# WU-CVGL/VicaSplat

Hardware: AMD Instinct MI355X
Metric: scenes/sec (8-view 256x256) encode+rasterize (higher is better)
Workload: dtype f32 (f32 activations; products as 3 x f16 MFMA on hi+lo operand pairs, f32 accumulate); 1 GPU; re10k_8view full pipeline fwd: ViT-L encoder+decoder+DPT heads -> 524288 Gaussians/scene, 12 target views/scene rasterized at 256x256; scenes_per_gpu=24, context_views=8, target_views=12, parallelism=scene-sharded x1 (no collective)

## Files before the change

### include/vicasplat_hip.h

```cpp
#ifndef VICASPLAT_HIP_H
#define VICASPLAT_HIP_H

#include <stddef.h>
#include <stdint.h>

#ifdef __cplusplus
extern "C" {
#endif

typedef void *vs_stream_t;

const char *vs_last_error(void);
int vs_abi_version(void);

typedef struct VsRasterIn {
    int32_t num_cameras;
    int32_t num_scenes;
    int32_t P;
    int32_t sh_degree;
    int32_t sh_coeffs;
    int32_t width, height;
    int32_t flags;
    const float *means3D;
    const float *cov3D;
// ... 63 lines not shown

int vs_rope2d(void *tokens, const int64_t *pos, int32_t B, int32_t N, int32_t H, int32_t D, int64_t sB, int64_t sN,
              float base, float fwd, int32_t dtype, vs_stream_t stream);


int vs_split_pack_weight(const float *w, int64_t ldw, void *out, int64_t ldo, int32_t N, int32_t K, int32_t scale_exp, vs_stream_t stream);

int vs_gemm_split(const float *A, const void *Wp, float acc_scale, const float *bias, float *out, const float *gate, const float *resid,
                  int32_t M, int32_t N, int32_t K, int32_t lda, int32_t ldw, int32_t ldo, int32_t epilogue, int32_t grp_in, int32_t grp_out,
                  int32_t grp_off, int32_t gate_rows, int32_t gate_ld, int32_t a_grp_in, int32_t a_grp_out, int32_t a_grp_off,
                  const int32_t *pos, const uint8_t *kind, int32_t C, float base2d, float theta1d, vs_stream_t stream);

int vs_conv3x3_split_res2_nhwc(const float *in, const void *wp, float acc_scale, const float *bias, const float *residual, const float *residual2,
                               float *out, int32_t Nimg, int32_t Hin, int32_t Win, int32_t Cin, int32_t Cout, int32_t stride, int32_t relu_in,
                               int32_t relu_out, vs_stream_t stream);
int vs_gemm_split_packed(const void *Ap, const void *Wp, float acc_scale, const float *bias, float *out, const float *gate, const float *resid,
                         int32_t M, int32_t N, int32_t K, int32_t lda, int32_t ldw, int32_t ldo, int32_t epilogue, int32_t grp_in, int32_t grp_out,
                         int32_t grp_off, int32_t gate_rows, int32_t gate_ld, int32_t a_grp_in, int32_t a_grp_out, int32_t a_grp_off,
                         const int32_t *pos, const uint8_t *kind, int32_t C, float base2d, float theta1d, vs_stream_t stream);
int vs_conv7x7_rgb_split_nhwc(const float *in_padded, const void *wp, float acc_scale, const float *bias, float *out, int32_t Nimg, int32_t H,
                              int32_t W, int32_t Hp, int32_t Wp, int32_t Cout, vs_stream_t stream);
int vs_conv7x7_rgb_split_up_nhwc(const float *in_padded, const void *wp, float acc_scale, const float *bias, const float *up_src, void *out_packed,
                                 int32_t Nimg, int32_t H, int32_t W, int32_t Hp, int32_t Wp, int32_t Cout, vs_stream_t stream);

int vs_conv3x3_head_dot_split_nhwc(const float *in, const void *wp, float acc_scale, const float *bias, const float *w2, const float *bias2,
                                   float *out2, int32_t Nimg, int32_t H, int32_t W, int32_t Cin, int32_t C2, int32_t ld2, int32_t relu_in,
                                   int32_t relu_out, vs_stream_t stream);

int vs_conv3x3_head1x1_split_nhwc(const float *in, const void *wp, float acc_scale, const float *bias, const void *w2p, float acc_scale2,
                                  const float *bias2, float *out2, int32_t Nimg, int32_t H, int32_t W, int32_t Cin, int32_t C2, int32_t C2pad,
// ... 155 lines not shown
```

### vicasplat_amd/_lib.py

```python
from __future__ import annotations

import ctypes as C
import os
import subprocess
import threading

import torch

_HERE = os.path.dirname(os.path.abspath(__file__))
_SO = os.environ.get("VICASPLAT_HIP_LIB") or os.path.join(_HERE, "libvicasplat_hip.so")
_lock = threading.Lock()
ABI_VERSION = 8
_lib = None

VS_BUF_GEOM, VS_BUF_RECT, VS_BUF_CLAMPED, VS_BUF_TILE_RANGES, VS_BUF_TILE_CURSOR, VS_BUF_KEYS, VS_BUF_POINT_LIST, \
    VS_BUF_SORT_SCRATCH, VS_BUF_FINAL_T, VS_BUF_N_CONTRIB, VS_BUF_MISC, VS_BUF_DEPTH, VS_BUF_CHECKPOINT, VS_BUF_COUNT = range(14)
VS_RASTER_COUNT_TOUCHED = 1
VS_RASTER_SAVE_FOR_BACKWARD = 2
VS_RASTER_SH_RGB_MAJOR = 4
VS_RASTER_COV_3X3 = 8

AllocFn = C.CFUNCTYPE(C.c_void_p, C.c_void_p, C.c_int32, C.c_size_t)


class VsRasterIn(C.Structure):
    _fields_ = [
        ("num_cameras", C.c_int32), ("num_scenes", C.c_int32), ("P", C.c_int32), ("sh_degree", C.c_int32),
# ... 121 lines not shown
            L.vs_linear_f32.argtypes = [vp, i64, vp, i64, vp, vp, i64, i32, i32, i32, i32, vp]
            L.vs_silu_cast.restype = C.c_int
            L.vs_silu_cast.argtypes = [vp, vp, i64, i32, vp]
            L.vs_conv3x3_head1x1_nhwc.restype = C.c_int
            L.vs_conv3x3_head1x1_nhwc.argtypes = [vp, vp, vp, vp, vp, vp] + [i32] * 11 + [vp]
            L.vs_split_pack_weight.restype = C.c_int
            L.vs_split_pack_weight.argtypes = [vp, i64, vp, i64, i32, i32, i32, vp]
            L.vs_gemm_split.restype = C.c_int
            L.vs_gemm_split.argtypes = [vp, vp, f32, vp, vp, vp, vp] + [i32] * 15 + [vp, vp, i32, f32, f32, vp]
            L.vs_gemm_split_packed.restype = C.c_int
            L.vs_gemm_split_packed.argtypes = [vp, vp, f32, vp, vp, vp, vp] + [i32] * 15 + [vp, vp, i32, f32, f32, vp]
            L.vs_conv3x3_split_nhwc.restype = C.c_int
            L.vs_conv3x3_split_nhwc.argtypes = [vp, vp, f32, vp, vp, vp] + [i32] * 8 + [vp]
            L.vs_conv3x3_split_res2_nhwc.restype = C.c_int
            L.vs_conv3x3_split_res2_nhwc.argtypes = [vp, vp, f32, vp, vp, vp, vp] + [i32] * 8 + [vp]
            L.vs_conv3x3_head1x1_split_nhwc.restype = C.c_int
            L.vs_conv3x3_head1x1_split_nhwc.argtypes = [vp, vp, f32, vp, vp, f32, vp, vp] + [i32] * 8 + [vp]
            L.vs_conv3x3_head_dot_split_nhwc.restype = C.c_int
            L.vs_conv3x3_head_dot_split_nhwc.argtypes = [vp, vp, f32, vp, vp, vp, vp] + [i32] * 8 + [vp]
            L.vs_conv7x7_rgb_split_nhwc.restype = C.c_int
            L.vs_conv7x7_rgb_split_nhwc.argtypes = [vp, vp, f32, vp, vp, i32, i32, i32, i32, i32, i32, vp]
            L.vs_conv7x7_rgb_split_up_nhwc.restype = C.c_int
            L.vs_conv7x7_rgb_split_up_nhwc.argtypes = [vp, vp, f32, vp, vp, vp, i32, i32, i32, i32, i32, i32, vp]
            L.vs_upsample2x_nhwc.restype = C.c_int
            L.vs_upsample2x_nhwc.argtypes = [vp, vp, vp, i32, i32, i32, i32, i32, i32, vp]
            L.vs_probe_mfma_rate.restype = C.c_int
            L.vs_probe_mfma_rate.argtypes = [vp, vp, i32, C.POINTER(C.c_double), vp]
            L.vs_transpose_f32.restype = C.c_int
            L.vs_transpose_f32.argtypes = [vp, i64, vp, i64, i32, i32, i32, i32, i32, i32, i32, i32, vp, vp]
            L.vs_gemm_wgrad_split_atn.restype = C.c_int
# ... 67 lines not shown
```

### vicasplat_amd/csrc/api.hip

```cpp
#include "common.h"

namespace vs {
static thread_local char g_err[512] = "";
void set_error(const char *fmt, ...) {
    va_list ap;
    va_start(ap, fmt);
    vsnprintf(g_err, sizeof(g_err), fmt, ap);
    va_end(ap);
}
}

extern "C" const char *vs_last_error(void) { return vs::g_err; }
extern "C" int vs_abi_version(void) { return 8; }

namespace {
typedef _Float16 half8p __attribute__((ext_vector_type(8)));
typedef float f4p __attribute__((ext_vector_type(4)));
__global__ void __launch_bounds__(256) mfma_rate_kernel(const half8p *__restrict__ in, float *__restrict__ out, int iters) {
    const int t = blockIdx.x * 256 + threadIdx.x;
    half8p a[4], b[4];
#pragma unroll
    for (int i = 0; i < 4; ++i) { a[i] = in[(t * 8 + i) & 65535]; b[i] = in[(t * 8 + 4 + i) & 65535]; }
    f4p c[16];
#pragma unroll
    for (int i = 0; i < 16; ++i) c[i] = f4p{0.f, 0.f, 0.f, 0.f};
    for (int it = 0; it < iters; ++it) {
#pragma unroll
        for (int i = 0; i < 4; ++i)
// ... 19 lines not shown
```

### vicasplat_amd/csrc/conv.hip

```cpp
#include "gemm256.h"

#include <cstdlib>

__device__ __attribute__((aligned(128))) unsigned short vs_zero_page[64] = {0};

namespace {

struct ConvArgs {
    const unsigned short *in;
    const unsigned short *w;
    const float *bias;
    const unsigned short *res;
    unsigned short *out;
    int Nimg, H, W, Cin, Cout;
    int relu_in, relu_out;
    int Hin, Win, stride;
    const unsigned short *w2;
    const float *bias2;
    unsigned short *out2;
    int C2, C2pad, ld2;
    float acc_scale;
    float acc_scale2;
    int a_packed;
    const float *res2;
    int korder;
};

static int conv_korder() {
    static const int v = [] { const char *e = getenv("VS_CONV_KORDER"); return e ? atoi(e) : 1; }();
    return v;
}

template <int BF16, int MI>
__device__ __forceinline__ void conv_epilogue(const ConvArgs &g, f4 (&acc)[MI][4], int mw0, int nbase, int M, void *, int, int lane) {
    const int mrow = lane & 15, c4 = (lane >> 4) * 4;
    if constexpr (BF16 == kDtSplit) {
#pragma unroll
        for (int i = 0; i < MI; ++i)
#pragma unroll
            for (int j = 0; j < 4; ++j) acc[i][j] *= g.acc_scale;
// ... 46 lines not shown
                } else {
                    unsigned short *dst = g.out + (size_t)(mw0 + (odd ? i : i - 1) * 16 + mrow) * g.Cout + nbase + (c4 & ~4);
#pragma unroll
                    for (int j = 0; j < 4; ++j) {
                        const u2v_ sx = __builtin_amdgcn_permlane16_swap(prev[j].x, pk[j].x, false, false);
                        const u2v_ sy = __builtin_amdgcn_permlane16_swap(prev[j].y, pk[j].y, false, false);
                        *reinterpret_cast<uint4 *>(dst + j * 16) = make_uint4(sx.x, sy.x, sx.y, sy.y);
                    }
                }
            }
            return;
        }
    }
    if constexpr (is_f32io(BF16)) {
        if (g.Cout % 4 == 0 && nbase + 64 <= g.Cout && mw0 + 16 * MI <= M &&
            ((reinterpret_cast<uintptr_t>(g.out) | reinterpret_cast<uintptr_t>(g.res) | reinterpret_cast<uintptr_t>(g.res2)) & 15) == 0) {
            const float *res32 = reinterpret_cast<const float *>(g.res);
            float *out32 = reinterpret_cast<float *>(g.out);
#pragma unroll
            for (int i = 0; i < MI; ++i) {
                const size_t o = (size_t)(mw0 + i * 16 + mrow) * g.Cout + nbase + c4;
                float4 rv[4];
                if (res32) {
#pragma unroll
                    for (int j = 0; j < 4; ++j) rv[j] = *reinterpret_cast<const float4 *>(res32 + o + j * 16);
                }
#pragma unroll
                for (int j = 0; j < 4; ++j) {
                    float v[4];
#pragma unroll
                    for (int r = 0; r < 4; ++r) v[r] = acc[i][j][r] + bv[j][r];
                    if (res32) {
                        const float rr[4] = {rv[j].x, rv[j].y, rv[j].z, rv[j].w};
#pragma unroll
                        for (int r = 0; r < 4; ++r) v[r] = g.relu_out == 2 ? (rr[r] > 0.f ? v[r] : 0.f) : v[r] + rr[r];
                    }
                    if (g.res2) {
                        const float4 r2 = *reinterpret_cast<const float4 *>(g.res2 + o + j * 16);
                        v[0] += r2.x; v[1] += r2.y; v[2] += r2.z; v[3] += r2.w;
                    }
                    if (g.relu_out == 1) {
#pragma unroll
                        for (int r = 0; r < 4; ++r) v[r] = fmaxf(v[r], 0.0f);
                    }
                    *reinterpret_cast<float4 *>(out32 + o + j * 16) = make_float4(v[0], v[1], v[2], v[3]);
                }
            }
            return;
        }
    }
#pragma unroll
    for (int i = 0; i < MI; ++i) {
        const int m = mw0 + i * 16 + mrow;
        if (m >= M) continue;
        const size_t o = (size_t)m * g.Cout + nbase + c4;
#pragma unroll
        for (int j = 0; j < 4; ++j) {
            float v[4];
#pragma unroll
            for (int r = 0; r < 4; ++r) v[r] = acc[i][j][r] + bv[j][r];
            if constexpr (is_f32io(BF16)) {
                const float *res32 = reinterpret_cast<const float *>(g.res);
                float *out32 = reinterpret_cast<float *>(g.out);
#pragma unroll
                for (int r = 0; r < 4; ++r)
                    if (nbase + j * 16 + c4 + r < g.Cout) {
                        float x = v[r];
                        if (res32) {
                            const float rr = res32[o + j * 16 + r];
                            x = g.relu_out == 2 ? (rr > 0.f ? x : 0.f) : x + rr;
                        }
                        if (g.res2) x += g.res2[o + j * 16 + r];
                        if (g.relu_out == 1) x = fmaxf(x, 0.0f);
                        v[r] = x;
                    }
                if (nbase + j * 16 + c4 + 3 < g.Cout && g.Cout % 4 == 0) {
                    *reinterpret_cast<float4 *>(out32 + o + j * 16) = make_float4(v[0], v[1], v[2], v[3]);
                } else {
#pragma unroll
                    for (int r = 0; r < 4; ++r)
                        if (nbase + j * 16 + c4 + r < g.Cout) out32[o + j * 16 + r] = v[r];
                }
                continue;
            }
            constexpr int D16 = is_f32io(BF16) ? 0 : BF16;
            if (vec_ok) {
                if (g.res) {
                    const uint2 rv = *reinterpret_cast<const uint2 *>(g.res + o + j * 16);
                    const float r0 = from16<D16>((unsigned short)(rv.x & 0xffffu)), r1 = from16<D16>((unsigned short)(rv.x >> 16));
                    const float r2 = from16<D16>((unsigned short)(rv.y & 0xffffu)), r3 = from16<D16>((unsigned short)(rv.y >> 16));
                    if (g.relu_out == 2) {
                        v[0] = r0 > 0.f ? v[0] : 0.f; v[1] = r1 > 0.f ? v[1] : 0.f; v[2] = r2 > 0.f ? v[2] : 0.f; v[3] = r3 > 0.f ? v[3] : 0.f;
                    } else {
                        v[0] += r0; v[1] += r1; v[2] += r2; v[3] += r3;
                    }
                }
// ... 546 lines not shown
#pragma unroll
            for (int j = 0; j < 4; ++j) {
                const int rb_ = wc * 64 + j * 16 + frow;
                fbh[j] = *reinterpret_cast<const uint4 *>(&cW0[rb_ * 32 + ((fg ^ swz4(rb_)) << 3)]);
                fbl[j] = *reinterpret_cast<const uint4 *>(&cW1[rb_ * 32 + ((fg ^ swz4(rb_)) << 3)]);
            }
#pragma unroll
            for (int i = 0; i < MI; ++i) {
                const int ra_ = wr * (16 * MI) + i * 16 + frow;
                uint4 fa0 = *reinterpret_cast<const uint4 *>(&cA0[ra_ * 32 + ((fg ^ swz4(ra_)) << 3)]);
                uint4 fa1 = *reinterpret_cast<const uint4 *>(&cA1[ra_ * 32 + ((fg ^ swz4(ra_)) << 3)]);
                if (g.relu_in) {
                    fa0.x = relu_reg<BF16>(fa0.x); fa0.y = relu_reg<BF16>(fa0.y); fa0.z = relu_reg<BF16>(fa0.z); fa0.w = relu_reg<BF16>(fa0.w);
                    fa1.x = relu_reg<BF16>(fa1.x); fa1.y = relu_reg<BF16>(fa1.y); fa1.z = relu_reg<BF16>(fa1.z); fa1.w = relu_reg<BF16>(fa1.w);
                }
                split8(fa0, fa1);
#pragma unroll
                for (int j = 0; j < 4; ++j) acc[i][j] = mma2<BF16>(fbh[j], fbl[j], fa0, fa1, acc[i][j]);
            }
        }
    } else {
        VS_STAGE(0)
        if (nk > 1) VS_STAGE(1)
        for (int kt = 0; kt < nk; kt += 3) {
            VS_STEP(kt, 0, 2)
            if (kt + 1 < nk) VS_STEP(kt + 1, 1, 0)
            if (kt + 2 < nk) VS_STEP(kt + 2, 2, 1)
        }
    }
#undef VS_STEP
#undef VS_STAGE
// ... 199 lines not shown
                acc[2 * k] += wgt * from16<BF16>((unsigned short)(vv[k] & 0xffffu));
                acc[2 * k + 1] += wgt * from16<BF16>((unsigned short)(vv[k] >> 16));
            }
        }
    }
    unsigned r[4];
#pragma unroll
    for (int k = 0; k < 4; ++k) r[k] = pack16x2<BF16>(acc[2 * k], acc[2 * k + 1]);
    *reinterpret_cast<uint4 *>(din + ((((size_t)n * H + y) * W + x) * C + cc * 8)) = make_uint4(r[0], r[1], r[2], r[3]);
}

}

static int conv3x3_entry(const void *in, const void *w, const float *bias, const void *residual, void *out, int32_t Nimg,
                         int32_t Hin, int32_t Win, int32_t Cin, int32_t Cout, int32_t stride, int32_t relu_in, int32_t relu_out,
                         int32_t dtype, float acc_scale, vs_stream_t stream_, const float *residual2 = nullptr) {
    const int H = (Hin - 1) / (stride > 0 ? stride : 1) + 1, W = (Win - 1) / (stride > 0 ? stride : 1) + 1;
    hipStream_t stream = (hipStream_t)stream_;
    VS_CHECK(in && w && out, "vs_conv3x3_nhwc: null pointer");
    VS_CHECK(Nimg >= 0 && Hin > 0 && Win > 0 && Cin > 0 && Cout > 0 && (stride == 1 || stride == 2), "vs_conv3x3_nhwc: bad sizes");
    VS_CHECK(dtype == 1 || dtype == 2 || dtype == 3 || dtype == 4, "vs_conv3x3_nhwc: dtype must be 1 (f16), 2 (bf16), 3 (f32) or 4 (split)");
    if (dtype == 3 || dtype == 4) {
        VS_CHECK(Cin % 16 == 0, "vs_conv3x3_nhwc: Cin=%d must be a multiple of 16 for f32 (pad the channels)", Cin);
        Cin *= 2;
    }
    VS_CHECK(Cin % 32 == 0, "vs_conv3x3_nhwc: Cin=%d must be a multiple of 32 (pad the channels)", Cin);
    VS_CHECK(Hin < 32767 && Win < 65536 && (long long)Nimg * Hin * Win < 2147483647LL, "vs_conv3x3_nhwc: image too large");
    VS_CHECK(relu_out >= 0 && relu_out <= 2 && (relu_out != 2 || residual), "vs_conv3x3_nhwc: relu_out must be 0, 1 or 2 (2 = mask by `residual`, which must be given)");
    VS_CHECK(((uintptr_t)in & 15) == 0 && ((uintptr_t)w & 15) == 0, "vs_conv3x3_nhwc: 16-byte alignment required");
    if (Nimg == 0) return 0;
    const int in_packed = (relu_in & 16) ? 1 : 0;
    relu_in &= ~16;
    VS_CHECK(!in_packed || (dtype == 4 && relu_in == 0), "vs_conv3x3_split_nhwc: a packed input is a split-class operand that carries its ReLU already");
    ConvArgs g{(const unsigned short *)in, (const unsigned short *)w, bias, (const unsigned short *)residual, (unsigned short *)out,
               Nimg, H, W, Cin, Cout, relu_in, relu_out, Hin, Win, stride, nullptr, nullptr, nullptr, 0, 0, 0, acc_scale, 1.f, in_packed, residual2};
    g.korder = conv_korder();
    VS_CHECK(!residual2 || ((dtype == 3 || dtype == 4) && relu_out != 2), "vs_conv3x3_nhwc: a second residual needs f32 activations (dtype 3 / 4) and no mask epilogue");
    const long long M = (long long)Nimg * H * W;
    static const int force = [] { const char *e = getenv("VS_CONV_MI"); return e ? atoi(e) : 0; }();
    int cshift = -1;
    for (int sft = 0; sft < 4; ++sft)
        if (Cin == (64 << sft)) cshift = sft;
    const int kpt_any = (Cin % 64 == 0 && Cin / 64 <= 64) ? Cin / 64 : -1;
    const long long t256 = vs::cdiv64(M, 256) * vs::cdiv(Cout, 256);
    static const int t256_min_env = [] { const char *e = getenv("VS_CONV_T256_MIN"); return e ? atoi(e) : 0; }();
    const long long t256_min = t256_min_env > 0 ? t256_min_env : (dtype == 4 ? 150 : 224);
    if (force != 8 && force != 4 && dtype == 4 && cshift < 0 && kpt_any > 0 && Cout % 256 == 0 && (9 * kpt_any) % 2 == 0 && t256 >= t256_min && !g.a_packed) {
        dim3 grid((unsigned)t256), block(512);
        if (relu_in) hipLaunchKernelGGL((conv3x3_256_kernel<kDtSplit, true>), grid, block, 0, stream, g, kpt_any);
        else hipLaunchKernelGGL((conv3x3_256_kernel<kDtSplit, false>), grid, block, 0, stream, g, kpt_any);
        VS_HIP(hipGetLastError());
        return 0;
    }
    if (force != 8 && force != 4 && cshift >= 0 && Cout % 256 == 0 && (9 * Cin / 64) % 2 == 0 && t256 >= t256_min) {
        dim3 grid((unsigned)t256), block(512);
        if (dtype == 4) {
            if (g.a_packed) hipLaunchKernelGGL((conv3x3_256_kernel<kDtSplit, false, 0, true>), grid, block, 0, stream, g, 1 << cshift);
            else if (relu_in) hipLaunchKernelGGL((conv3x3_256_kernel<kDtSplit, true>), grid, block, 0, stream, g, 1 << cshift);
            else hipLaunchKernelGGL((conv3x3_256_kernel<kDtSplit, false>), grid, block, 0, stream, g, 1 << cshift);
        } else if (dtype == 3) {
            if (relu_in) hipLaunchKernelGGL((conv3x3_256_kernel<kDtF32, true>), grid, block, 0, stream, g, 1 << cshift);
            else hipLaunchKernelGGL((conv3x3_256_kernel<kDtF32, false>), grid, block, 0, stream, g, 1 << cshift);
        } else if (dtype == 2) {
            if (relu_in) hipLaunchKernelGGL((conv3x3_256_kernel<true, true>), grid, block, 0, stream, g, 1 << cshift);
// ... 5 lines not shown
        VS_HIP(hipGetLastError());
        return 0;
    }
    const long long big = vs::cdiv64(M, 256) * vs::cdiv(Cout, BN);
    if (dtype == 4) {
        VS_CHECK(Cin % 64 == 0, "vs_conv3x3_split_nhwc: Cin must be a multiple of 32");
        static const int no128 = [] { const char *e = getenv("VS_CONV_SPLIT_NO256X128"); return e ? atoi(e) : 0; }();
        if (!no128 && cshift >= 0 && Cout % 128 == 0 && Cout % 256 != 0 && (9 * Cin / 64) % 2 == 0 && big >= 224) {
            dim3 grid((unsigned)(vs::cdiv64(M, 256) * (Cout / 128))), block(512);
            if (g.a_packed) hipLaunchKernelGGL((conv3x3_256x128_split_kernel<false, false, true>), grid, block, 0, stream, g, 1 << cshift);
            else if (relu_in) hipLaunchKernelGGL((conv3x3_256x128_split_kernel<true, false>), grid, block, 0, stream, g, 1 << cshift);
            else hipLaunchKernelGGL((conv3x3_256x128_split_kernel<false, false>), grid, block, 0, stream, g, 1 << cshift);
            VS_HIP(hipGetLastError());
            return 0;
        }
        VS_CHECK(!g.a_packed, "vs_conv3x3_split_nhwc: a packed input is taken by the 256 x 256 and 256 x 128 tile kernels only (this shape runs on the 4-wave kernel)");
        static const int smi = [] { const char *e = getenv("VS_CONV_SPLIT_MI"); return e ? atoi(e) : 0; }();
        static const int mi2 = [] { const char *e = getenv("VS_CONV_MI2"); return e ? atoi(e) : 1; }();
        const long long t4 = vs::cdiv64(M, 128) * vs::cdiv(Cout, BN);
        if ((big >= 512 && smi != 4) || smi == 8) hipLaunchKernelGGL((conv3x3_kernel<kDtSplit, 8>), dim3((unsigned)big), dim3(256), 0, stream, g);
        else if (mi2 && smi == 0 && t4 <= 192 && M > 64) hipLaunchKernelGGL((conv3x3_kernel<kDtSplit, 2>), dim3((unsigned)(vs::cdiv64(M, 64) * vs::cdiv(Cout, BN))), dim3(256), 0, stream, g);
        else hipLaunchKernelGGL((conv3x3_kernel<kDtSplit, 4>), dim3((unsigned)t4), dim3(256), 0, stream, g);
    } else if (dtype == 3) {
        hipLaunchKernelGGL((conv3x3_kernel<kDtF32, 4>), dim3((unsigned)(vs::cdiv64(M, 128) * vs::cdiv(Cout, BN))), dim3(256), 0, stream, g);
    } else if ((big >= 256 || force == 8) && force != 4) {
        dim3 grid((unsigned)big);
        if (dtype == 2) hipLaunchKernelGGL((conv3x3_kernel<true, 8>), grid, dim3(256), 0, stream, g);
        else hipLaunchKernelGGL((conv3x3_kernel<false, 8>), grid, dim3(256), 0, stream, g);
    } else {
        dim3 grid((unsigned)(vs::cdiv64(M, 128) * vs::cdiv(Cout, BN)));
        if (dtype == 2) hipLaunchKernelGGL((conv3x3_kernel<true, 4>), grid, dim3(256), 0, stream, g);
// ... 10 lines not shown
    return conv3x3_entry(in, w, bias, residual, out, Nimg, Hin, Win, Cin, Cout, stride, relu_in, relu_out, dtype, 1.f, stream_);
}

extern "C" int vs_conv3x3_split_nhwc(const float *in, const void *wp, float acc_scale, const float *bias, const float *residual, float *out,
                                     int32_t Nimg, int32_t Hin, int32_t Win, int32_t Cin, int32_t Cout, int32_t stride, int32_t relu_in,
                                     int32_t relu_out, vs_stream_t stream_) {
    VS_CHECK(acc_scale > 0.f && Cin % 32 == 0, "vs_conv3x3_split_nhwc: acc_scale must be positive and Cin a multiple of 32");
    return conv3x3_entry(in, wp, bias, residual, out, Nimg, Hin, Win, Cin, Cout, stride, relu_in, relu_out, 4, acc_scale, stream_);
}

extern "C" int vs_conv3x3_split_res2_nhwc(const float *in, const void *wp, float acc_scale, const float *bias, const float *residual,
                                          const float *residual2, float *out, int32_t Nimg, int32_t Hin, int32_t Win, int32_t Cin, int32_t Cout,
                                          int32_t stride, int32_t relu_in, int32_t relu_out, vs_stream_t stream_) {
    VS_CHECK(acc_scale > 0.f && Cin % 32 == 0, "vs_conv3x3_split_res2_nhwc: acc_scale must be positive and Cin a multiple of 32");
    return conv3x3_entry(in, wp, bias, residual, out, Nimg, Hin, Win, Cin, Cout, stride, relu_in, relu_out, 4, acc_scale, stream_, residual2);
}

extern "C" int vs_conv3x3_head1x1_nhwc(const void *in, const void *w, const float *bias, const void *w2, const float *bias2, void *out2,
                                       int32_t Nimg, int32_t H, int32_t W, int32_t Cin, int32_t Cout, int32_t C2, int32_t C2pad, int32_t ld2,
                                       int32_t relu_in, int32_t relu_out, int32_t dtype, vs_stream_t stream_) {
    hipStream_t stream = (hipStream_t)stream_;
    VS_CHECK(in && w && w2 && bias2 && out2, "vs_conv3x3_head1x1_nhwc: null pointer");
    VS_CHECK(dtype == 1 || dtype == 2, "vs_conv3x3_head1x1_nhwc: dtype must be 1 (f16) or 2 (bf16)");
    VS_CHECK(Nimg > 0 && H > 0 && W > 0 && H < 32767 && W < 65536, "vs_conv3x3_head1x1_nhwc: bad sizes");
    const long long M = (long long)Nimg * H * W;
    VS_CHECK(M % 256 == 0 && M < 2147483647LL, "vs_conv3x3_head1x1_nhwc: N*H*W must be a multiple of 256");
    VS_CHECK(((uintptr_t)in & 15) == 0 && ((uintptr_t)w & 15) == 0 && ((uintptr_t)w2 & 15) == 0 && ((uintptr_t)out2 & 7) == 0 &&
             ((uintptr_t)bias2 & 15) == 0, "vs_conv3x3_head1x1_nhwc: alignment");
    VS_CHECK(relu_out == 0 || relu_out == 1, "vs_conv3x3_head1x1_nhwc: relu_out must be 0 or 1");
    ConvArgs g{(const unsigned short *)in, (const unsigned short *)w, bias, nullptr, nullptr, Nimg, H, W, Cin, Cout, relu_in, relu_out, H, W, 1,
// ... 151 lines not shown
```

### vicasplat_amd/model/encoder/heads/dpt.py

```python
from __future__ import annotations

import torch
import torch.nn.functional as F
from torch import nn

import os

from .... import ops

_PTS_UP_PACKED = os.environ.get("VS_PTS_UP_PACKED", "1") != "0"
_STEM_STREAM = os.environ.get("VS_STEM_STREAM", "1") != "0"
_STEM_UP_FUSED = os.environ.get("VS_STEM_UP_FUSED", "1") != "0"


def _no_torch_forward(self, *a, **k):
    raise RuntimeError(f"{type(self).__name__} is a PARAMETER CONTAINER (the reference's state_dict names): the computation runs on the HIP "
                       "kernels driven by PixelwiseTaskWithDPT -- there is no PyTorch / MIOpen forward in vicasplat_amd")


class _RCU(nn.Module):
    forward = _no_torch_forward

    def __init__(self, c: int):
        super().__init__()
        self.conv1 = nn.Conv2d(c, c, 3, 1, 1, bias=True)
        self.conv2 = nn.Conv2d(c, c, 3, 1, 1, bias=True)

# ... 133 lines not shown
        wk = F.pad(c.weight.detach().float().flatten(1), (0, 160 - 147)).contiguous()
        if self.split:
            P = self._packed()
            if "stem.ws" not in P:
                P["stem.ws"] = ops.split_pack_weight(wk)
            wk = P["stem.ws"]
        bias = c.bias.detach().float().contiguous()
        out = torch.empty(N, H, W, wk.shape[0], dtype=torch.float32, device=frames.device)
        step = 8
        for i in range(0, N, step):
            cols = F.pad(F.unfold(frames[i:i + step].float(), 7, padding=3).transpose(1, 2), (0, 160 - 147)).reshape(-1, 160).contiguous()
            ops.gemm(cols, wk, bias, out[i:i + step].view(-1, wk.shape[0]), ops.EPI_STORE16)
        return out

    @staticmethod
    def _gemm1x1(x, P, name, n_out=None):
        w, b = P[name + ".w"], P[name + ".b"]
        lead = x.shape[:-1]
        a = x.reshape(-1, x.shape[-1])
        out = torch.empty(a.shape[0], w.shape[0], dtype=x.dtype, device=x.device)
        ops.gemm(a, w, b, out, ops.EPI_STORE16)
        return out.view(*lead, w.shape[0])

    @staticmethod
    def _rcu(x, P, name, extra=None):
        t = ops.conv3x3_nhwc(x, P[name + ".c1.w"], P[name + ".c1.b"], relu_in=True, relu_out=True)
        return ops.conv3x3_nhwc(t, P[name + ".c2.w"], P[name + ".c2.b"], residual=x, residual2=extra)

    def _fusion(self, P, r, x, skip=None, packed_out=False):
        if skip is not None:
            if self.split:
                x = self._rcu(skip, P, f"rf{r}.resConfUnit1", extra=x.contiguous())
            else:
                x = x + self._rcu(skip, P, f"rf{r}.resConfUnit1")
        return ops.upsample2x_nhwc(self._gemm1x1(self._rcu(x, P, f"rf{r}.resConfUnit2"), P, f"rf{r}.out"), packed=packed_out)

    def _trunk(self, tokens, gh: int, gw: int, packed_out: bool = False):
        P = self._packed()
        d = self.dpt
        dt = self.compute_dtype
        t = [tokens[h] for h in d.hooks]
        BT = t[0].shape[0]
        maps = [x.reshape(BT, gh, gw, x.shape[-1]).to(dt).contiguous() for x in t]
        def convT(x, name, k):
            y = self._gemm1x1(x, P, name)
            Cp = y.shape[-1] // (k * k)
            return y.view(BT, gh, gw, k, k, Cp).permute(0, 1, 3, 2, 4, 5).reshape(BT, gh * k, gw * k, Cp)
        l0 = convT(self._gemm1x1(maps[0], P, "ap0.0"), "ap0.1", 4)
        l1 = convT(self._gemm1x1(maps[1], P, "ap1.0"), "ap1.1", 2)
        l2 = self._gemm1x1(maps[2], P, "ap2.0")
        l3 = ops.conv3x3_nhwc(self._gemm1x1(maps[3], P, "ap3.0"), P["ap3.1.w"], P["ap3.1.b"], stride=2)
        l0, l1, l2, l3 = [ops.conv3x3_nhwc(l.contiguous(), P[f"rn{i}.w"], None) for i, l in enumerate((l0, l1, l2, l3))]
        p4 = self._fusion(P, 4, l3)[:, :l2.shape[1], :l2.shape[2]].contiguous()
        p3 = self._fusion(P, 3, p4, l2)
        p2 = self._fusion(P, 2, p3, l1)
        return self._fusion(P, 1, p2, l0, packed_out=packed_out), P

    def forward_pts3d_raw(self, tokens, gh: int, gw: int) -> torch.Tensor:
        nc = self.num_channels
        pk = _PTS_UP_PACKED and self.split and self.dpt.head[0].out_channels == 128 and self.dpt.head[0].in_channels in (64, 128, 256)
        x, P = self._trunk(tokens, gh, gw, packed_out=pk and (tokens[self.dpt.hooks[0]].shape[0] * 64 * gh * gw) >= 224 * 256)
        x = ops.conv3x3_nhwc(x, P["h0.w"], P["h0.b"])
        npix = x.shape[0] * 4 * x.shape[1] * x.shape[2]
        if _PTS_UP_PACKED and self.split and npix % 256 == 0 and x.shape[-1] == 128 and self.dpt.head[2].out_channels == 128:
            if "h4f32.w" not in P:
                c4 = self.dpt.head[4]
                P["h4f32.w"] = torch.nn.functional.pad(c4.weight.detach().float().flatten(1), (0, 0, 0, 4 - c4.out_channels)).contiguous()
                P["h4f32.b"] = torch.nn.functional.pad(c4.bias.detach().float(), (0, 4 - c4.out_channels)).contiguous()
            xp = ops.upsample2x_nhwc(x, packed=True)
            y = ops.conv3x3_head1x1_nhwc(xp, P["h2.w"], P["h2.b"], P["h4f32.w"], P["h4f32.b"], nc)
            return y[..., :nc].permute(0, 3, 1, 2)
# ... 68 lines not shown
```

### vicasplat_amd/ops.py

```python
from __future__ import annotations

import os
from typing import Optional

import torch

from . import _lib as L

_DT = {torch.float32: 0, torch.float16: 1, torch.bfloat16: 2}
_DTX = {torch.float32: 3, torch.float16: 1, torch.bfloat16: 2}
_OPERAND_DTYPES = (torch.float16, torch.bfloat16, torch.float32)
EPI_STORE16, EPI_GELU16, EPI_RESID32, EPI_STORE32 = 0, 1, 2, 3


class _RangeGuard:
    LIMIT = 65520.0
    SLOTS = 4096

    def __init__(self):
        self.enabled, self.flags, self.names = False, None, []

    def begin(self, device):
        self.enabled = True
        if self.flags is None or self.flags.device != torch.device(device):
# ... 377 lines not shown
    assert d_raw is None or d_raw.numel() == npix * (11 + 3 * d_sh)
    pl, gl = (pts.shape[-1] + 7) // 8 * 8, (gs.shape[-1] + 7) // 8 * 8
    d_pts = torch.empty(pts.shape[:-1] + (pl,), dtype=pts.dtype, device=dev)
    d_gs = torch.empty(gs.shape[:-1] + (gl,), dtype=gs.dtype, device=dev)
    act = {"bounded": 0, "exp": 1, "softplus": 2}[scale_act]
    with torch.cuda.device(dev):
        rc = L.lib().vs_gaussian_adapter_backward(L.ptr(pts), pts.shape[-1], L.ptr(gs), _DT[pts.dtype], npix, d_sh, L.ptr(sh_mask), act,
                                                  scale_min, scale_max, opacity_exponent, L.ptr(d_means), L.ptr(d_cov), L.ptr(d_harm),
                                                  L.ptr(d_op), L.ptr(d_raw), L.ptr(d_pts), pl, L.ptr(d_gs), gl, L.stream_ptr(dev))
    L.check(rc, "vs_gaussian_adapter_backward")
    return d_pts[..., :pts.shape[-1]], d_gs[..., :gs.shape[-1]]


def conv3x3_nhwc(x: torch.Tensor, w: torch.Tensor, bias: Optional[torch.Tensor] = None, residual: Optional[torch.Tensor] = None,
                 relu_in: bool = False, relu_out: bool = False, out: Optional[torch.Tensor] = None, stride: int = 1,
                 mask_by: Optional[torch.Tensor] = None, residual2: Optional[torch.Tensor] = None) -> torch.Tensor:
    if mask_by is not None:
        assert residual is None and not relu_out
        residual, relu_out = mask_by, 2
    split = isinstance(w, SplitWeight)
    xin_packed = isinstance(x, SplitWeight)
    if xin_packed:
        assert split and not relu_in and residual2 is None
        x = x.data
    dev = L.require_device(x, w.data if split else w, bias, residual, out)
    assert x.dim() == 4 and x.is_contiguous() and w.is_contiguous() and (x.dtype in _OPERAND_DTYPES or xin_packed)
    assert (split and x.dtype == (torch.int32 if xin_packed else torch.float32)) or (not split and x.dtype == w.dtype)
    N, H, W, Cin = x.shape
    Cout = w.shape[0]
    assert tuple(w.shape) == (Cout, 3, 3, Cin)
    Ho, Wo = (H - 1) // stride + 1, (W - 1) // stride + 1
# ... 9 lines not shown
            rc = L.lib().vs_conv3x3_split_res2_nhwc(L.ptr(x), L.ptr(w.data), w.acc_scale, L.ptr(bias), L.ptr(residual), L.ptr(residual2), L.ptr(out), N, H, W,
                                                    Cin, Cout, stride, int(relu_in), int(relu_out), L.stream_ptr(dev))
        L.check(rc, "vs_conv3x3_split_res2_nhwc")
        return out
    if split:
        with torch.cuda.device(dev):
            rc = L.lib().vs_conv3x3_split_nhwc(L.ptr(x), L.ptr(w.data), w.acc_scale, L.ptr(bias), L.ptr(residual), L.ptr(out), N, H, W, Cin, Cout,
                                               stride, int(relu_in) | (16 if xin_packed else 0), int(relu_out), L.stream_ptr(dev))
        L.check(rc, "vs_conv3x3_split_nhwc")
        return out
    with torch.cuda.device(dev):
        rc = L.lib().vs_conv3x3_nhwc(L.ptr(x), L.ptr(w), L.ptr(bias), L.ptr(residual), L.ptr(out), N, H, W, Cin, Cout, stride,
                                     int(relu_in), int(relu_out), _DTX[x.dtype], L.stream_ptr(dev))
    L.check(rc, "vs_conv3x3_nhwc")
    return out


def conv3x3_head1x1_nhwc(x: torch.Tensor, w: torch.Tensor, bias: Optional[torch.Tensor], w2: torch.Tensor, bias2: torch.Tensor, n_out: int,
                         relu_out: bool = True) -> torch.Tensor:
    if isinstance(w, SplitWeight) and isinstance(w2, SplitWeight):
        xin_packed = isinstance(x, SplitWeight)
        if xin_packed:
            x = x.data
        dev = L.require_device(x, w.data, bias, w2.data, bias2)
        N, H, W, Cin = x.shape
        c2pad = w2.shape[0]
        assert x.is_contiguous() and x.dtype == (torch.int32 if xin_packed else torch.float32) and tuple(w.shape) == (256, 3, 3, Cin) and tuple(w2.shape) == (c2pad, 256)
        assert bias2.dtype == torch.float32 and bias2.numel() == c2pad and n_out <= c2pad
        out = torch.empty((N, H, W, c2pad), dtype=torch.float32, device=dev)
        if RANGE_GUARD.enabled:
# ... 804 lines not shown
```

Measured before the change: 101.4 scenes/s.

## Run DPT trunk on pre-split packed activations with dual f32/packed conv epilogues

Adds a conv3x3 entry point whose epilogue writes the output already split into hi/lo f16 pairs, optionally after applying ReLU, alongside or instead of the f32 output. The DPT trunk (reassemble 1x1s, layer_rn convs, refinenet RCUs) is rewired so each consumer receives packed operands and skips its own split and ReLU prologue; the 256-tile kernel now accepts packed inputs. This removes the repeated per-tile splitting of activations and some f32 round trips. In exchange, some layers write both a f32 and a packed copy, and the path adds more kernel variants and layout constraints.

```diff
diff --git a/include/vicasplat_hip.h b/include/vicasplat_hip.h
--- a/include/vicasplat_hip.h
+++ b/include/vicasplat_hip.h
@@ -101,6 +101,9 @@
 int vs_conv3x3_split_res2_nhwc(const float *in, const void *wp, float acc_scale, const float *bias, const float *residual, const float *residual2,
                                float *out, int32_t Nimg, int32_t Hin, int32_t Win, int32_t Cin, int32_t Cout, int32_t stride, int32_t relu_in,
                                int32_t relu_out, vs_stream_t stream);
+int vs_conv3x3_split_pk_nhwc(const float *in, const void *wp, float acc_scale, const float *bias, const float *residual, const float *residual2,
+                             float *out, void *out_packed, int32_t Nimg, int32_t Hin, int32_t Win, int32_t Cin, int32_t Cout, int32_t stride,
+                             int32_t relu_in, int32_t relu_out, int32_t relu_packed, vs_stream_t stream);
 int vs_gemm_split_packed(const void *Ap, const void *Wp, float acc_scale, const float *bias, float *out, const float *gate, const float *resid,
                          int32_t M, int32_t N, int32_t K, int32_t lda, int32_t ldw, int32_t ldo, int32_t epilogue, int32_t grp_in, int32_t grp_out,
                          int32_t grp_off, int32_t gate_rows, int32_t gate_ld, int32_t a_grp_in, int32_t a_grp_out, int32_t a_grp_off,
diff --git a/vicasplat_amd/_lib.py b/vicasplat_amd/_lib.py
--- a/vicasplat_amd/_lib.py
+++ b/vicasplat_amd/_lib.py
@@ -10,7 +10,7 @@
 _HERE = os.path.dirname(os.path.abspath(__file__))
 _SO = os.environ.get("VICASPLAT_HIP_LIB") or os.path.join(_HERE, "libvicasplat_hip.so")
 _lock = threading.Lock()
-ABI_VERSION = 8
+ABI_VERSION = 9
 _lib = None
 
 VS_BUF_GEOM, VS_BUF_RECT, VS_BUF_CLAMPED, VS_BUF_TILE_RANGES, VS_BUF_TILE_CURSOR, VS_BUF_KEYS, VS_BUF_POINT_LIST, \
@@ -162,6 +162,8 @@
             L.vs_conv3x3_split_nhwc.argtypes = [vp, vp, f32, vp, vp, vp] + [i32] * 8 + [vp]
             L.vs_conv3x3_split_res2_nhwc.restype = C.c_int
             L.vs_conv3x3_split_res2_nhwc.argtypes = [vp, vp, f32, vp, vp, vp, vp] + [i32] * 8 + [vp]
+            L.vs_conv3x3_split_pk_nhwc.restype = C.c_int
+            L.vs_conv3x3_split_pk_nhwc.argtypes = [vp, vp, f32, vp, vp, vp, vp, vp] + [i32] * 9 + [vp]
             L.vs_conv3x3_head1x1_split_nhwc.restype = C.c_int
             L.vs_conv3x3_head1x1_split_nhwc.argtypes = [vp, vp, f32, vp, vp, f32, vp, vp] + [i32] * 8 + [vp]
             L.vs_conv3x3_head_dot_split_nhwc.restype = C.c_int
diff --git a/vicasplat_amd/csrc/api.hip b/vicasplat_amd/csrc/api.hip
--- a/vicasplat_amd/csrc/api.hip
+++ b/vicasplat_amd/csrc/api.hip
@@ -11,7 +11,7 @@
 }
 
 extern "C" const char *vs_last_error(void) { return vs::g_err; }
-extern "C" int vs_abi_version(void) { return 8; }
+extern "C" int vs_abi_version(void) { return 9; }
 
 namespace {
 typedef _Float16 half8p __attribute__((ext_vector_type(8)));
diff --git a/vicasplat_amd/csrc/conv.hip b/vicasplat_amd/csrc/conv.hip
--- a/vicasplat_amd/csrc/conv.hip
+++ b/vicasplat_amd/csrc/conv.hip
@@ -24,6 +24,8 @@
     int a_packed;
     const float *res2;
     int korder;
+    float *outp;
+    int relu_packed;
 };
 
 static int conv_korder() {
@@ -100,7 +102,8 @@
     }
     if constexpr (is_f32io(BF16)) {
         if (g.Cout % 4 == 0 && nbase + 64 <= g.Cout && mw0 + 16 * MI <= M &&
-            ((reinterpret_cast<uintptr_t>(g.out) | reinterpret_cast<uintptr_t>(g.res) | reinterpret_cast<uintptr_t>(g.res2)) & 15) == 0) {
+            ((reinterpret_cast<uintptr_t>(g.out) | reinterpret_cast<uintptr_t>(g.res) | reinterpret_cast<uintptr_t>(g.res2) |
+              reinterpret_cast<uintptr_t>(g.outp)) & 15) == 0) {
             const float *res32 = reinterpret_cast<const float *>(g.res);
             float *out32 = reinterpret_cast<float *>(g.out);
 #pragma unroll
@@ -111,25 +114,38 @@
 #pragma unroll
                     for (int j = 0; j < 4; ++j) rv[j] = *reinterpret_cast<const float4 *>(res32 + o + j * 16);
                 }
+                float v[4][4];
 #pragma unroll
                 for (int j = 0; j < 4; ++j) {
-                    float v[4];
-#pragma unroll
-                    for (int r = 0; r < 4; ++r) v[r] = acc[i][j][r] + bv[j][r];
+#pragma unroll
+                    for (int r = 0; r < 4; ++r) v[j][r] = acc[i][j][r] + bv[j][r];
                     if (res32) {
                         const float rr[4] = {rv[j].x, rv[j].y, rv[j].z, rv[j].w};
 #pragma unroll
-                        for (int r = 0; r < 4; ++r) v[r] = g.relu_out == 2 ? (rr[r] > 0.f ? v[r] : 0.f) : v[r] + rr[r];
+                        for (int r = 0; r < 4; ++r) v[j][r] = g.relu_out == 2 ? (rr[r] > 0.f ? v[j][r] : 0.f) : v[j][r] + rr[r];
                     }
                     if (g.res2) {
                         const float4 r2 = *reinterpret_cast<const float4 *>(g.res2 + o + j * 16);
-                        v[0] += r2.x; v[1] += r2.y; v[2] += r2.z; v[3] += r2.w;
+                        v[j][0] += r2.x; v[j][1] += r2.y; v[j][2] += r2.z; v[j][3] += r2.w;
                     }
                     if (g.relu_out == 1) {
 #pragma unroll
-                        for (int r = 0; r < 4; ++r) v[r] = fmaxf(v[r], 0.0f);
+                        for (int r = 0; r < 4; ++r) v[j][r] = fmaxf(v[j][r], 0.0f);
                     }
-                    *reinterpret_cast<float4 *>(out32 + o + j * 16) = make_float4(v[0], v[1], v[2], v[3]);
+                    if (out32) *reinterpret_cast<float4 *>(out32 + o + j * 16) = make_float4(v[j][0], v[j][1], v[j][2], v[j][3]);
+                }
+                if constexpr (BF16 == kDtSplit) {
+                    if (g.outp) {
+                        if (g.relu_packed) {
+#pragma unroll
+                            for (int j = 0; j < 4; ++j)
+#pragma unroll
+                                for (int r = 0; r < 4; ++r) v[j][r] = __uint_as_float(relu_f32_lds(__float_as_uint(v[j][r])));
+                        }
+                        float *rowp = g.outp + (size_t)(mw0 + i * 16 + mrow) * g.Cout;
+#pragma unroll
+                        for (int j = 0; j < 4; j += 2) store_split8(rowp, nbase + c4 + j * 16, v[j], v[j + 1]);
+                    }
                 }
             }
             return;
@@ -160,12 +176,22 @@
                         if (g.relu_out == 1) x = fmaxf(x, 0.0f);
                         v[r] = x;
                     }
-                if (nbase + j * 16 + c4 + 3 < g.Cout && g.Cout % 4 == 0) {
+                if (!out32) {
+                } else if (nbase + j * 16 + c4 + 3 < g.Cout && g.Cout % 4 == 0) {
                     *reinterpret_cast<float4 *>(out32 + o + j * 16) = make_float4(v[0], v[1], v[2], v[3]);
                 } else {
 #pragma unroll
                     for (int r = 0; r < 4; ++r)
                         if (nbase + j * 16 + c4 + r < g.Cout) out32[o + j * 16 + r] = v[r];
+                }
+                if constexpr (BF16 == kDtSplit) {
+                    if (g.outp && nbase + j * 16 + c4 + 3 < g.Cout) {
+                        if (g.relu_packed) {
+#pragma unroll
+                            for (int r = 0; r < 4; ++r) v[r] = __uint_as_float(relu_f32_lds(__float_as_uint(v[r])));
+                        }
+                        store_split4(g.outp + (size_t)m * g.Cout, nbase + j * 16 + c4, v[0], v[1], v[2], v[3]);
+                    }
                 }
                 continue;
             }
@@ -742,7 +768,7 @@
                     fa0.x = relu_reg<BF16>(fa0.x); fa0.y = relu_reg<BF16>(fa0.y); fa0.z = relu_reg<BF16>(fa0.z); fa0.w = relu_reg<BF16>(fa0.w);
                     fa1.x = relu_reg<BF16>(fa1.x); fa1.y = relu_reg<BF16>(fa1.y); fa1.z = relu_reg<BF16>(fa1.z); fa1.w = relu_reg<BF16>(fa1.w);
                 }
-                split8(fa0, fa1);
+                if (!g.a_packed) split8(fa0, fa1);
 #pragma unroll
                 for (int j = 0; j < 4; ++j) acc[i][j] = mma2<BF16>(fbh[j], fbl[j], fa0, fa1, acc[i][j]);
             }
@@ -972,10 +998,13 @@
 
 static int conv3x3_entry(const void *in, const void *w, const float *bias, const void *residual, void *out, int32_t Nimg,
                          int32_t Hin, int32_t Win, int32_t Cin, int32_t Cout, int32_t stride, int32_t relu_in, int32_t relu_out,
-                         int32_t dtype, float acc_scale, vs_stream_t stream_, const float *residual2 = nullptr) {
+                         int32_t dtype, float acc_scale, vs_stream_t stream_, const float *residual2 = nullptr, float *out_packed = nullptr,
+                         int32_t relu_packed = 0) {
     const int H = (Hin - 1) / (stride > 0 ? stride : 1) + 1, W = (Win - 1) / (stride > 0 ? stride : 1) + 1;
     hipStream_t stream = (hipStream_t)stream_;
-    VS_CHECK(in && w && out, "vs_conv3x3_nhwc: null pointer");
+    VS_CHECK(in && w && (out || out_packed), "vs_conv3x3_nhwc: null pointer");
+    VS_CHECK(!out_packed || (dtype == 4 && Cout % 64 == 0 && ((uintptr_t)out_packed & 15) == 0 && relu_out != 2),
+             "vs_conv3x3_split_pk_nhwc: a packed output needs split operands, Cout %% 64 == 0, 16-byte alignment and no mask epilogue");
     VS_CHECK(Nimg >= 0 && Hin > 0 && Win > 0 && Cin > 0 && Cout > 0 && (stride == 1 || stride == 2), "vs_conv3x3_nhwc: bad sizes");
     VS_CHECK(dtype == 1 || dtype == 2 || dtype == 3 || dtype == 4, "vs_conv3x3_nhwc: dtype must be 1 (f16), 2 (bf16), 3 (f32) or 4 (split)");
     if (dtype == 3 || dtype == 4) {
@@ -993,6 +1022,8 @@
     ConvArgs g{(const unsigned short *)in, (const unsigned short *)w, bias, (const unsigned short *)residual, (unsigned short *)out,
                Nimg, H, W, Cin, Cout, relu_in, relu_out, Hin, Win, stride, nullptr, nullptr, nullptr, 0, 0, 0, acc_scale, 1.f, in_packed, residual2};
     g.korder = conv_korder();
+    g.outp = out_packed;
+    g.relu_packed = relu_packed ? 1 : 0;
     VS_CHECK(!residual2 || ((dtype == 3 || dtype == 4) && relu_out != 2), "vs_conv3x3_nhwc: a second residual needs f32 activations (dtype 3 / 4) and no mask epilogue");
     const long long M = (long long)Nimg * H * W;
     static const int force = [] { const char *e = getenv("VS_CONV_MI"); return e ? atoi(e) : 0; }();
@@ -1003,9 +1034,10 @@
     const long long t256 = vs::cdiv64(M, 256) * vs::cdiv(Cout, 256);
     static const int t256_min_env = [] { const char *e = getenv("VS_CONV_T256_MIN"); return e ? atoi(e) : 0; }();
     const long long t256_min = t256_min_env > 0 ? t256_min_env : (dtype == 4 ? 150 : 224);
-    if (force != 8 && force != 4 && dtype == 4 && cshift < 0 && kpt_any > 0 && Cout % 256 == 0 && (9 * kpt_any) % 2 == 0 && t256 >= t256_min && !g.a_packed) {
+    if (force != 8 && force != 4 && dtype == 4 && cshift < 0 && kpt_any > 0 && Cout % 256 == 0 && (9 * kpt_any) % 2 == 0 && t256 >= t256_min) {
         dim3 grid((unsigned)t256), block(512);
-        if (relu_in) hipLaunchKernelGGL((conv3x3_256_kernel<kDtSplit, true>), grid, block, 0, stream, g, kpt_any);
+        if (g.a_packed) hipLaunchKernelGGL((conv3x3_256_kernel<kDtSplit, false, 0, true>), grid, block, 0, stream, g, kpt_any);
+        else if (relu_in) hipLaunchKernelGGL((conv3x3_256_kernel<kDtSplit, true>), grid, block, 0, stream, g, kpt_any);
         else hipLaunchKernelGGL((conv3x3_256_kernel<kDtSplit, false>), grid, block, 0, stream, g, kpt_any);
         VS_HIP(hipGetLastError());
         return 0;
@@ -1041,7 +1073,6 @@
             VS_HIP(hipGetLastError());
             return 0;
         }
-        VS_CHECK(!g.a_packed, "vs_conv3x3_split_nhwc: a packed input is taken by the 256 x 256 and 256 x 128 tile kernels only (this shape runs on the 4-wave kernel)");
         static const int smi = [] { const char *e = getenv("VS_CONV_SPLIT_MI"); return e ? atoi(e) : 0; }();
         static const int mi2 = [] { const char *e = getenv("VS_CONV_MI2"); return e ? atoi(e) : 1; }();
         const long long t4 = vs::cdiv64(M, 128) * vs::cdiv(Cout, BN);
@@ -1082,6 +1113,15 @@
                                           int32_t stride, int32_t relu_in, int32_t relu_out, vs_stream_t stream_) {
     VS_CHECK(acc_scale > 0.f && Cin % 32 == 0, "vs_conv3x3_split_res2_nhwc: acc_scale must be positive and Cin a multiple of 32");
     return conv3x3_entry(in, wp, bias, residual, out, Nimg, Hin, Win, Cin, Cout, stride, relu_in, relu_out, 4, acc_scale, stream_, residual2);
+}
+
+extern "C" int vs_conv3x3_split_pk_nhwc(const float *in, const void *wp, float acc_scale, const float *bias, const float *residual,
+                                        const float *residual2, float *out, void *out_packed, int32_t Nimg, int32_t Hin, int32_t Win, int32_t Cin,
+                                        int32_t Cout, int32_t stride, int32_t relu_in, int32_t relu_out, int32_t relu_packed, vs_stream_t stream_) {
+    VS_CHECK(acc_scale > 0.f && Cin % 32 == 0, "vs_conv3x3_split_pk_nhwc: acc_scale must be positive and Cin a multiple of 32");
+    VS_CHECK(out_packed, "vs_conv3x3_split_pk_nhwc: null packed output (use vs_conv3x3_split_res2_nhwc)");
+    return conv3x3_entry(in, wp, bias, residual, out, Nimg, Hin, Win, Cin, Cout, stride, relu_in, relu_out, 4, acc_scale, stream_, residual2,
+                         (float *)out_packed, relu_packed);
 }
 
 extern "C" int vs_conv3x3_head1x1_nhwc(const void *in, const void *w, const float *bias, const void *w2, const float *bias2, void *out2,
diff --git a/vicasplat_amd/model/encoder/heads/dpt.py b/vicasplat_amd/model/encoder/heads/dpt.py
--- a/vicasplat_amd/model/encoder/heads/dpt.py
+++ b/vicasplat_amd/model/encoder/heads/dpt.py
@@ -11,6 +11,7 @@
 _PTS_UP_PACKED = os.environ.get("VS_PTS_UP_PACKED", "1") != "0"
 _STEM_STREAM = os.environ.get("VS_STEM_STREAM", "1") != "0"
 _STEM_UP_FUSED = os.environ.get("VS_STEM_UP_FUSED", "1") != "0"
+_TRUNK_PACKED = os.environ.get("VS_TRUNK_PACKED", "1") != "0"
 
 
 def _no_torch_forward(self, *a, **k):
@@ -174,13 +175,42 @@
         return out
 
     @staticmethod
-    def _gemm1x1(x, P, name, n_out=None):
+    def _gemm1x1(x, P, name, n_out=None, packed_out=False):
         w, b = P[name + ".w"], P[name + ".b"]
-        lead = x.shape[:-1]
-        a = x.reshape(-1, x.shape[-1])
-        out = torch.empty(a.shape[0], w.shape[0], dtype=x.dtype, device=x.device)
+        if isinstance(x, ops.SplitWeight):
+            lead, K, dev = x.data.shape[:-1], x.data.shape[-1], x.data.device
+            a, odt = ops.SplitWeight(x.data.reshape(-1, K), 1.0, (x.data.numel() // K, K)), torch.float32
+        else:
+            lead, dev, odt = x.shape[:-1], x.device, x.dtype
+            a = x.reshape(-1, x.shape[-1])
+        M = a.shape[0]
+        if packed_out:
+            out = torch.empty(M, w.shape[0], dtype=torch.int32, device=dev)
+            ops.gemm(a, w, b, ops.SplitWeight(out, 1.0, out.shape), ops.EPI_STORE16)
+            out = out.view(*lead, w.shape[0])
+            return ops.SplitWeight(out, 1.0, out.shape)
+        out = torch.empty(M, w.shape[0], dtype=odt, device=dev)
         ops.gemm(a, w, b, out, ops.EPI_STORE16)
         return out.view(*lead, w.shape[0])
+
+    @staticmethod
+    def _relu_dual(x, w, b, residual=None, extra=None, stride=1):
+        xd = x.data if isinstance(x, ops.SplitWeight) else x
+        Ho, Wo = (xd.shape[1] - 1) // stride + 1, (xd.shape[2] - 1) // stride + 1
+        yr = ops.empty_packed((xd.shape[0], Ho, Wo, w.shape[0]), xd.device)
+        return ops.conv3x3_nhwc(x, w, b, residual=residual, residual2=extra, stride=stride, packed_relu_out=yr), yr
+
+    def _rcu_packed(self, x, xr, P, name, extra=None, last=False):
+        t = ops.conv3x3_nhwc(xr, P[name + ".c1.w"], P[name + ".c1.b"], relu_out=True, packed_out=True)
+        if last:
+            return ops.conv3x3_nhwc(t, P[name + ".c2.w"], P[name + ".c2.b"], residual=x, residual2=extra, packed_out=True)
+        return self._relu_dual(t, P[name + ".c2.w"], P[name + ".c2.b"], residual=x, extra=extra)
+
+    def _fusion_packed(self, P, r, x, xr, skip=None, skip_r=None, packed_out=False):
+        if skip is not None:
+            x, xr = self._rcu_packed(skip, skip_r, P, f"rf{r}.resConfUnit1", extra=x.contiguous())
+        y = self._rcu_packed(x, xr, P, f"rf{r}.resConfUnit2", last=True)
+        return ops.upsample2x_nhwc(self._gemm1x1(y, P, f"rf{r}.out"), packed=packed_out)
 
     @staticmethod
     def _rcu(x, P, name, extra=None):
@@ -202,6 +232,14 @@
         t = [tokens[h] for h in d.hooks]
         BT = t[0].shape[0]
         maps = [x.reshape(BT, gh, gw, x.shape[-1]).to(dt).contiguous() for x in t]
+        def convT(x, name, k):
+            y = self._gemm1x1(x, P, name)
+            Cp = y.shape[-1] // (k * k)
+            return y.view(BT, gh, gw, k, k, Cp).permute(0, 1, 3, 2, 4, 5).reshape(BT, gh * k, gw * k, Cp)
+        feat = d.scratch.layer1_rn.out_channels
+        if (_TRUNK_PACKED and self.split and feat % 64 == 0 and P["ap3.1.w"].shape[0] % 64 == 0
+                and all(P[f"rn{i}.w"].shape[-1] % 32 == 0 for i in range(4))):
+            return self._trunk_packed(P, maps, BT, gh, gw, packed_out), P
         def convT(x, name, k):
             y = self._gemm1x1(x, P, name)
             Cp = y.shape[-1] // (k * k)
@@ -215,6 +253,22 @@
         p3 = self._fusion(P, 3, p4, l2)
         p2 = self._fusion(P, 2, p3, l1)
         return self._fusion(P, 1, p2, l0, packed_out=packed_out), P
+
+    def _trunk_packed(self, P, maps, BT, gh, gw, packed_out):
+        def convT(x, name, k):
+            y = self._gemm1x1(x, P, name, packed_out=True).data
+            Cp = y.shape[-1] // (k * k)
+            y = y.view(BT, gh, gw, k, k, Cp).permute(0, 1, 3, 2, 4, 5).reshape(BT, gh * k, gw * k, Cp).contiguous()
+            return ops.SplitWeight(y, 1.0, y.shape)
+        l0 = convT(self._gemm1x1(maps[0], P, "ap0.0", packed_out=True), "ap0.1", 4)
+        l1 = convT(self._gemm1x1(maps[1], P, "ap1.0", packed_out=True), "ap1.1", 2)
+        l2 = self._gemm1x1(maps[2], P, "ap2.0", packed_out=True)
+        l3 = ops.conv3x3_nhwc(self._gemm1x1(maps[3], P, "ap3.0", packed_out=True), P["ap3.1.w"], P["ap3.1.b"], stride=2, packed_out=True)
+        (l0, r0), (l1, r1), (l2, r2), (l3, r3) = [self._relu_dual(l, P[f"rn{i}.w"], None) for i, l in enumerate((l0, l1, l2, l3))]
+        p4 = self._fusion_packed(P, 4, l3, r3)[:, :l2.shape[1], :l2.shape[2]].contiguous()
+        p3 = self._fusion_packed(P, 3, p4, None, l2, r2)
+        p2 = self._fusion_packed(P, 2, p3, None, l1, r1)
+        return self._fusion_packed(P, 1, p2, None, l0, r0, packed_out=packed_out)
 
     def forward_pts3d_raw(self, tokens, gh: int, gw: int) -> torch.Tensor:
         nc = self.num_channels
diff --git a/vicasplat_amd/ops.py b/vicasplat_amd/ops.py
--- a/vicasplat_amd/ops.py
+++ b/vicasplat_amd/ops.py
@@ -415,7 +415,11 @@
 
 def conv3x3_nhwc(x: torch.Tensor, w: torch.Tensor, bias: Optional[torch.Tensor] = None, residual: Optional[torch.Tensor] = None,
                  relu_in: bool = False, relu_out: bool = False, out: Optional[torch.Tensor] = None, stride: int = 1,
-                 mask_by: Optional[torch.Tensor] = None, residual2: Optional[torch.Tensor] = None) -> torch.Tensor:
+                 mask_by: Optional[torch.Tensor] = None, residual2: Optional[torch.Tensor] = None, packed_out: bool = False,
+                 packed_relu_out: Optional["SplitWeight"] = None):
+    if packed_out or packed_relu_out is not None:
+        assert out is None and mask_by is None
+        return _conv3x3_split_pk(x, w, bias, residual, residual2, relu_in, relu_out, stride, packed_out, packed_relu_out)
     if mask_by is not None:
         assert residual is None and not relu_out
         residual, relu_out = mask_by, 2
@@ -455,6 +459,40 @@
                                      int(relu_in), int(relu_out), _DTX[x.dtype], L.stream_ptr(dev))
     L.check(rc, "vs_conv3x3_nhwc")
     return out
+
+
+def empty_packed(shape, device) -> SplitWeight:
+    return SplitWeight(torch.empty(tuple(shape), dtype=torch.int32, device=device), 1.0, tuple(shape))
+
+
+def _conv3x3_split_pk(x, w, bias, residual, residual2, relu_in, relu_out, stride, packed_only, relu_pk):
+    assert isinstance(w, SplitWeight) and not (packed_only and relu_pk is not None) and not (relu_pk is not None and relu_out)
+    xin_packed = isinstance(x, SplitWeight)
+    if xin_packed:
+        assert not relu_in and x.acc_scale == 1.0
+        x = x.data
+    dev = L.require_device(x, w.data, bias, residual, residual2)
+    assert x.dim() == 4 and x.is_contiguous() and x.dtype == (torch.int32 if xin_packed else torch.float32)
+    N, H, W, Cin = x.shape
+    Cout = w.shape[0]
+    assert tuple(w.shape) == (Cout, 3, 3, Cin) and Cout % 64 == 0
+    Ho, Wo = (H - 1) // stride + 1, (W - 1) // stride + 1
+    for r in (residual, residual2):
+        assert r is None or (r.shape == (N, Ho, Wo, Cout) and r.is_contiguous() and r.dtype == torch.float32)
+    if RANGE_GUARD.enabled:
+        RANGE_GUARD.check(f"conv3x3 {Cin}->{Cout} @{H}x{W}", SplitWeight(x.view(-1, Cin), 1.0, (N * H * W, Cin)) if xin_packed else x)
+    if packed_only:
+        outp, out = torch.empty((N, Ho, Wo, Cout), dtype=torch.int32, device=dev), None
+    else:
+        outp, out = relu_pk.data, torch.empty((N, Ho, Wo, Cout), dtype=torch.float32, device=dev)
+        assert relu_pk.acc_scale == 1.0 and outp.dtype == torch.int32 and outp.is_contiguous() and tuple(outp.shape) == (N, Ho, Wo, Cout)
+        L.require_device(outp, out)
+    with torch.cuda.device(dev):
+        rc = L.lib().vs_conv3x3_split_pk_nhwc(L.ptr(x), L.ptr(w.data), w.acc_scale, L.ptr(bias), L.ptr(residual), L.ptr(residual2), L.ptr(out),
+                                              L.ptr(outp), N, H, W, Cin, Cout, stride, int(relu_in) | (16 if xin_packed else 0), int(relu_out),
+                                              int(not packed_only), L.stream_ptr(dev))
+    L.check(rc, "vs_conv3x3_split_pk_nhwc")
+    return SplitWeight(outp, 1.0, outp.shape) if packed_only else out
 
 
 def conv3x3_head1x1_nhwc(x: torch.Tensor, w: torch.Tensor, bias: Optional[torch.Tensor], w2: torch.Tensor, bias2: torch.Tensor, n_out: int,
```

Measured after the change: 102.6 scenes/s, median of 6. 1.01x the previous value.
